# cuMF/cumf_als

Hardware: AMD Instinct MI355X
Metric: ratings/sec per ALS half-iteration (Netflix f=100); RMSE vs reference (higher is better)
Workload: dtype f32 (bf16x3-split products on the bf16 matrix pipe, fp32 accumulate); 1 GPU; netflix-shape synthetic ratings 17770x480189, nnz=99072112, f=100, lambda=0.048, solver=lu, X_BATCH=1 THETA_BATCH=1, fused Gram+solve; step=update-X + update-Theta (two half-iterations)

## Files before the change

cumf_als_amd/csrc/als_internal.h:

```cpp
#ifndef CUMF_ALS_INTERNAL_H_
#define CUMF_ALS_INTERNAL_H_

#include <hip/hip_runtime.h>

#include <algorithm>
#include <cstddef>
#include <type_traits>

#ifndef CUMF_ABLATE
#define CUMF_ABLATE 0
#endif

namespace cumf {

constexpr int kThreads = 256;
constexpr int kStage = 32;
constexpr int kVecLd = 128;
constexpr int kMaxFusedNB = 9;
constexpr int kMaxF = 207;
constexpr int kMaxFAny = 512;
constexpr int kMaxWaveNB = 7;
constexpr int kMaxFusedLuWaveNB = 9;

enum { kModeCG = 0, kModeLU = 1, kModeMaterialize = 2, kModeLUExact = 3, kModeCGHalf = 4 };

__host__ __device__ constexpr int nb_for_f(int f) { return f / 16 + 1; }
constexpr int kMaxNB = nb_for_f(kMaxF);
__host__ __device__ constexpr int solve_ldg(int f, int mode) { return mode == kModeCG ? ((f + 1 + 3) & ~3) : (f + 1); }
__host__ __device__ constexpr size_t solve_g_floats(int f, int mode) {
  return ((size_t)f * solve_ldg(f, mode) + 3) & ~(size_t)3;
}
__host__ __device__ constexpr size_t lu_packed_floats(int nb) { return (size_t)256 * nb * (nb + 1) / 2 + 16 * nb; }
__host__ __device__ constexpr size_t lu_lds_floats(int nb, int f) { return lu_packed_floats(nb) + (size_t)((f + 3) & ~3) + 48; }
constexpr int kCgExtraFloats = 12 * kVecLd;
__host__ __device__ constexpr size_t solve_lds_floats(int f, int mode) {
  return solve_g_floats(f, mode) + (mode == kModeCG ? (size_t)kCgExtraFloats : 0);
}

__host__ __device__ constexpr bool fused_supported(int f, int mode) {
  return mode == kModeLU ? nb_for_f(f) <= nb_for_f(kMaxF) : (f <= kVecLd && nb_for_f(f) <= kMaxFusedNB);
}

struct KernelArgs {
  const int* item_row;
  const long long* item_begin;
  const int* item_len;
  const int* item_slot;
  const int* item_rowlen;
  const int* mrow_row;
  const int* mrow_slot0;
  const int* mrow_nslots;
  const int* mrow_rowlen;
  float* part;
  const int* colidx;
  const float* val;
  const float* gather;
  float* update;
  float* tt;
  float* rhs;
  int tt_half;
  int tt_packed;
  int dense_slots;
  int whole_only;
  long long row_begin;
  int f;
  float lambda;
  int cg_iters;
  int dbg;
  int fast_words;
  int* fast_flag;
  int pre_words;
  unsigned pre_pitch;
  double* sse_bins;
  const float* gather_f32;
  int no_pack;
};
constexpr int kSseBins = 1024;

struct PlanLists {
  long n_items, n_mrows;
  long n_citems, n_witems;
  const int *c_row, *c_len, *c_slot, *c_rowlen;
  const long long* c_begin;
  const int *w_row, *w_len, *w_rowlen;
  const long long* w_begin;
  float* part2;
  long part2_rows;
  double chunk_share;
  long n_short;
};
constexpr int kShortRow = 32;
bool short_cg_available(int f);
hipError_t launch_short_cg(const KernelArgs& a, long n_items, hipStream_t stream);
hipError_t launch_solve_batched(const float* A, const float* b, float* x, long batch, int f, int mode, int cg_iters,
                                hipStream_t stream);
enum { kGramAuto = 0, kGramExact = 1, kGramFast = 2 };
enum { kArithSplit3 = 0, kArithFast = 1, kArithPre = 2, kArithPrePk = 3, kArithSplitPk = 4 };

struct Switches {
  int gram;
  int presplit;
  double presplit_mb;
  bool splitpk;
  bool short_cg;
  bool batched;
  bool wave_solve;
  bool lu_exact;
};
Switches switches();
void set_gram_mode(int mode);
void set_presplit_mode(int mode);

struct PlanFacts {
  int nb;
  long n_mrows, n_citems, n_witems;
  double chunk_share;
  long n_short;
  long gather_rows;
};
enum Path {
  kPathNone,
  kPathGeneric,
  kPathWorkgroup,
  kPathOneWave,
  kPathTwoWave,
};
enum Table { kTableNone, kTablePlanes, kTableF16Words };
enum Solve {
  kSolveInKernel,
  kSolveTileBuffer,
  kSolveReduce,
  kSolveWaveCG,
};
struct Route {
  Path path;
  int arith;
  int fc;
  Table table;
  bool chunk_first;
  long n_short;
  Solve chunked;
  Solve whole;
  bool sse;
};
Route route_for(int f, int mode, const PlanFacts& plan, const Switches& sw);
hipError_t launch_half_iteration(const KernelArgs& a, int mode, const Route& r, const PlanLists& lists, hipStream_t stream);

hipError_t launch_presplit(const float* src, unsigned* dst, size_t n, int* flag, hipStream_t stream);
hipError_t launch_gram_generic(const KernelArgs& a, long n_items, hipStream_t stream);
hipError_t launch_lu_global(float* A, const float* b, float* x, long batch, int f, hipStream_t stream);
__host__ __device__ constexpr bool presplit_supported(int f) {
  return ((nb_for_f(f) == 7 || nb_for_f(f) == 5) && ((f & 15) == 0 || (f & 15) == 4)) ||
         (nb_for_f(f) > kMaxWaveNB && nb_for_f(f) <= nb_for_f(kMaxF) && (f & 3) == 0 && (f & 15) <= 8);
}
__host__ __device__ constexpr bool presplit_pays(int f) { return presplit_supported(f) && nb_for_f(f) >= 7; }
__host__ __device__ constexpr bool presplit_pays_any_size(int f) { return presplit_supported(f) && nb_for_f(f) >= 10; }
__host__ __device__ constexpr unsigned presplit_pitch(int f) {
  return 96u * (f / 16) + ((f & 15) ? (nb_for_f(f) > kMaxWaveNB ? 64u : 32u) : 0u);
}
hipError_t launch_presplit3(const float* src, void* dst, long long rows, int f, hipStream_t stream);
hipError_t launch_pack_upper(const float* full, float* packed, long batch, int f, int unpack, hipStream_t stream);
void set_last_error(int code);
void set_kernel_timing(bool on);
void note_item_kernel(const void* host_function);
const void* last_item_kernel();
hipError_t last_kernel_ms(float* item_ms, float* reduce_ms);
hipError_t kernel_ms_since_reset(float* item_ms, float* reduce_ms, int* launches);
hipError_t launch_quadratic_terms(const float* A, const float* b, const float* x, const float* reg, long batch, int f,
                                  double* out, hipStream_t stream);
hipError_t launch_sse(const float* val, const int* row, const int* col, const float* thetaT, const float* XT,
                      long count, int f, int surpass_nan, double* out, hipStream_t stream);
hipError_t launch_cg_global(const float* A, const float* b, float* x, long batch, int f, int cg_iters, bool a_half,
                            hipStream_t stream);

template <int NB>
hipError_t slice_half_iteration(const KernelArgs& a, int mode, long n_items, long n_mrows, hipStream_t stream);
template <int NB>
hipError_t slice_solve(const float* A, const float* b, float* x, long batch, int f, int mode, int cg_iters,
                       hipStream_t stream);
template <int NB>
hipError_t slice_reduce_only(const KernelArgs& a, int mode, const Route& r, long n_mrows, hipStream_t stream);
template <int NB>
hipError_t slice_batched(const KernelArgs& a, int mode, const Route& r, const PlanLists& L, hipStream_t stream);
template <int NB>
hipError_t wave_item_launch(const KernelArgs& a, int mode, const Route& r, bool whole, long n_items, hipStream_t stream);
template <int NB>
hipError_t wave_solve_launch(const KernelArgs& a, int mode, long n_rows, hipStream_t stream);
template <int NB>
hipError_t wave_lu_launch(const KernelArgs& a, const Route& r, bool whole, long n_items, hipStream_t stream);
template <int NB>
hipError_t wave_cg_hist(unsigned long long* out16);

template <int LO, int HI, class Go>
hipError_t with_nb(int nb, Go&& go) {
  if constexpr (LO > HI)
    return hipErrorInvalidValue;
  else
    return nb == LO ? go(std::integral_constant<int, LO>{}) : with_nb<LO + 1, HI>(nb, go);
}

#define CUMF_LOCAL __attribute__((visibility("hidden")))

enum {
  kScratchTiles = 0,
  kScratchWords = 1,
  kScratchPlanes = 2,
  kScratchImpGram = 3,
  kScratchImpSlots = 4,
  kScratchImpTT = 5,
  kScratchImpRhs = 6,
  kScratchImpX = 7,
  kScratchImpAux = 8,
  kScratchTopkWork = 9,
  kScratchTopkPart = 10,
  kScratchTopkMetrics = 11,
  kScratchNnlsTT = 12,
  kScratchNnlsRhs = 13,
  kScratchRankKeys = 14,
  kScratchRankHist = 15,
  kScratchRankValid = 16,
  kScratchRankMetrics = 17,
};
int scratch_get(hipStream_t stream, int kind, size_t bytes, void** out);
template <typename T>
CUMF_LOCAL inline int scratch(hipStream_t stream, int kind, size_t count, T** out) {
  void* q = nullptr;
  const int rc = scratch_get(stream, kind, (count ? count : 1) * sizeof(T), &q);
  *out = static_cast<T*>(q);
  return rc;
}
CUMF_LOCAL size_t scratch_capacity(hipStream_t stream, int kind);
CUMF_LOCAL int fast_flag_get(int** out);
struct ScratchLease {
  int dev = 0;
  ScratchLease();
  ~ScratchLease();
  ScratchLease(const ScratchLease&) = delete;
  ScratchLease& operator=(const ScratchLease&) = delete;
};
struct ImplicitLists;
void free_implicit_lists(ImplicitLists* lists);

}

struct cumf_plan {
  long rows = 0, row_begin = 0, row_end = 0;
  int f = 0, nb = 0, chunk = 0;
  long long plan_nnz = 0;
  long long chunk_nnz = 0;
  long n_items = 0, n_slots = 0, n_mrows = 0;
  long n_short = 0;
  int* d_item_row = nullptr;
  long long* d_item_begin = nullptr;
  int* d_item_len = nullptr;
  int* d_item_slot = nullptr;
  int* d_item_rowlen = nullptr;
  int* d_mrow_row = nullptr;
  int* d_mrow_slot0 = nullptr;
  int* d_mrow_nslots = nullptr;
  int* d_mrow_rowlen = nullptr;
  float* d_part = nullptr;
  char* d_block = nullptr;
  long n_citems = 0, n_witems = 0;
  int *d_c_row = nullptr, *d_c_len = nullptr, *d_c_slot = nullptr, *d_c_rowlen = nullptr;
  long long* d_c_begin = nullptr;
  int *d_w_row = nullptr, *d_w_len = nullptr, *d_w_rowlen = nullptr;
  long long* d_w_begin = nullptr;
  long gather_rows = 0;
  cumf::ImplicitLists* implicit = nullptr;
};

namespace cumf {

CUMF_LOCAL int plan_lists(const cumf_plan* p, PlanLists* out, hipStream_t stream, bool need_tiles);
CUMF_LOCAL PlanFacts plan_facts(const cumf_plan* p);

template <bool NOTE = false, typename... P, typename... A>
hipError_t launch_kernel(void (*kernel)(P...), dim3 grid, dim3 block, size_t lds, hipStream_t stream, const A&... args) {
  const void* fn = reinterpret_cast<const void*>(kernel);
  if (lds > 64 * 1024) {
    hipError_t e = hipFuncSetAttribute(fn, hipFuncAttributeMaxDynamicSharedMemorySize, (int)lds);
    if (e != hipSuccess) return e;
  }
  if (NOTE) note_item_kernel(fn);
  hipLaunchKernelGGL(kernel, grid, block, lds, stream, args...);
  return hipGetLastError();
}
template <typename... P, typename... A>
hipError_t launch_item_kernel(void (*kernel)(P...), dim3 grid, dim3 block, size_t lds, hipStream_t stream,
                              const A&... args) {
  return launch_kernel<true>(kernel, grid, block, lds, stream, args...);
}

}

#define CUMF_HIP_CHECK(call)                                                                          \
  do {                                                                                                \
    hipError_t err__ = (call);                                                                        \
    if (err__ != hipSuccess) {                                                                        \
      fprintf(stderr, "HIP Error:\nFile = %s\nLine = %d\nReason = %s\n", __FILE__, __LINE__,          \
              hipGetErrorString(err__));                                                              \
      return (int)err__;                                                                              \
    }                                                                                                 \
  } while (0)

#endif
```

cumf_als_amd/csrc/als_launch.cpp:

```cpp
#include <atomic>
#include <mutex>
#include <vector>

#include "als_internal.h"

namespace cumf {

namespace {
struct TimedLaunch {
  hipEvent_t ev[3];
  bool item, reduce;
};
constexpr size_t kTimedPool = 1024;
bool g_timing = false;
std::vector<TimedLaunch> g_timed;
size_t g_timed_used = 0;
TimedLaunch* g_newest = nullptr;
std::mutex g_timed_mutex;

TimedLaunch* timing_begin() {
  if (!g_timing) return nullptr;
  std::lock_guard<std::mutex> lock(g_timed_mutex);
  if (g_timed_used == kTimedPool) g_timed_used = 0;
  g_newest = &g_timed[g_timed_used++];
  return g_newest;
}

std::atomic<const void*> g_last_item_kernel{nullptr};
}

void set_kernel_timing(bool on) {
  std::lock_guard<std::mutex> lock(g_timed_mutex);
  g_timing = on;
  if (on && g_timed.empty()) {
    g_timed.resize(kTimedPool);
    for (auto& t : g_timed) {
      for (auto& e : t.ev) (void)hipEventCreate(&e);
      t.item = t.reduce = false;
    }
  }
}
hipError_t last_kernel_ms(float* item_ms, float* reduce_ms) {
  *item_ms = 0.f;
  *reduce_ms = 0.f;
  const TimedLaunch* t = g_newest;
  if (!t) return hipSuccess;
  hipError_t e = hipEventSynchronize(t->ev[2]);
  if (e != hipSuccess) return e;
  if (t->item) (void)hipEventElapsedTime(item_ms, t->ev[0], t->ev[1]);
  if (t->reduce) (void)hipEventElapsedTime(reduce_ms, t->ev[1], t->ev[2]);
  return hipSuccess;
}
hipError_t kernel_ms_since_reset(float* item_ms, float* reduce_ms, int* launches) {
  std::lock_guard<std::mutex> lock(g_timed_mutex);
  *item_ms = 0.f;
  *reduce_ms = 0.f;
  *launches = (int)g_timed_used;
  for (size_t i = 0; i < g_timed_used; ++i) {
    TimedLaunch& t = g_timed[i];
    hipError_t e = hipEventSynchronize(t.ev[2]);
    if (e != hipSuccess) return e;
    float ms = 0.f;
    if (t.item && hipEventElapsedTime(&ms, t.ev[0], t.ev[1]) == hipSuccess) *item_ms += ms;
    if (t.reduce && hipEventElapsedTime(&ms, t.ev[1], t.ev[2]) == hipSuccess) *reduce_ms += ms;
  }
  g_timed_used = 0;
  return hipSuccess;
}

void note_item_kernel(const void* host_function) { g_last_item_kernel.store(host_function, std::memory_order_relaxed); }
const void* last_item_kernel() { return g_last_item_kernel.load(std::memory_order_relaxed); }

static hipError_t wave_items(const KernelArgs& a, int mode, const Route& r, bool whole, long n_items, hipStream_t stream) {
  return with_nb<2, kMaxWaveNB>(nb_for_f(a.f), [&](auto nb) { return wave_item_launch<nb>(a, mode, r, whole, n_items, stream); });
}

static hipError_t one_wave_items(const KernelArgs& a, int mode, const Route& r, const PlanLists& L, hipStream_t stream) {
  KernelArgs aw = a;
  long n_items = L.n_items;
  if (r.chunk_first) {
    aw.item_row = L.w_row, aw.item_begin = L.w_begin, aw.item_len = L.w_len;
    aw.item_slot = nullptr, aw.item_rowlen = L.w_rowlen;
    n_items = L.n_witems;
  }
  if (r.n_short > 0) {
    n_items -= r.n_short;
    KernelArgs as = aw;
    as.item_row += n_items, as.item_begin += n_items, as.item_len += n_items, as.item_rowlen += n_items;
    hipError_t e = launch_short_cg(as, r.n_short, stream);
    if (e != hipSuccess) return e;
  }
  if (r.chunk_first) {
    KernelArgs ac = a;
    ac.item_row = L.c_row, ac.item_begin = L.c_begin, ac.item_len = L.c_len;
    ac.item_slot = L.c_slot, ac.item_rowlen = L.c_rowlen;
    hipError_t e = wave_items(ac, mode, r, false, L.n_citems, stream);
    if (e != hipSuccess) return e;
  }
  return wave_items(aw, mode, r, r.chunk_first || L.n_mrows == 0, n_items, stream);
}

hipError_t launch_half_iteration(const KernelArgs& a, int mode, const Route& r, const PlanLists& L, hipStream_t stream) {
  const int nb = nb_for_f(a.f);
  TimedLaunch* t = timing_begin();
  if (t) {
    t->item = r.path == kPathTwoWave || L.n_items > 0;
    t->reduce = r.path != kPathTwoWave && L.n_mrows > 0;
    (void)hipEventRecord(t->ev[0], stream);
  }
  hipError_t e = hipErrorInvalidValue;
  switch (r.path) {
    case kPathTwoWave:
      e = with_nb<kMaxWaveNB + 1, kMaxNB>(nb, [&](auto n) { return slice_batched<n>(a, mode, r, L, stream); });
      break;
    case kPathOneWave: e = one_wave_items(a, mode, r, L, stream); break;
    case kPathWorkgroup:
      e = with_nb<1, kMaxNB>(nb, [&](auto n) { return slice_half_iteration<n>(a, mode, L.n_items, 0, stream); });
      break;
    default: break;
  }
  if (t) (void)hipEventRecord(t->ev[1], stream);
  if (e == hipSuccess && r.path != kPathTwoWave && L.n_mrows > 0) {
    e = with_nb<1, kMaxNB>(nb, [&](auto n) {
      return r.path == kPathOneWave ? slice_reduce_only<n>(a, mode, r, L.n_mrows, stream)
                                    : slice_half_iteration<n>(a, mode, 0, L.n_mrows, stream);
    });
  }
  if (t) (void)hipEventRecord(t->ev[2], stream);
  return e;
}

hipError_t launch_solve_batched(const float* A, const float* b, float* x, long batch, int f, int mode, int cg_iters,
                                hipStream_t stream) {
  if (batch <= 0) return hipSuccess;
  if (mode == kModeLUExact) return slice_solve<0>(A, b, x, batch, f, mode, 0, stream);
  if (f > 128 && (mode == kModeCG || mode == kModeCGHalf))
    return launch_cg_global(A, b, x, batch, f, cg_iters, mode == kModeCGHalf, stream);
  return with_nb<1, kMaxNB>(nb_for_f(f), [&](auto n) { return slice_solve<n>(A, b, x, batch, f, mode, cg_iters, stream); });
}

}
```

cumf_als_amd/csrc/als_plan.cpp:

```cpp
#include <hip/hip_runtime.h>

#include <algorithm>
#include <cstdint>
#include <cstdio>
#include <cstdlib>
#include <numeric>
#include <vector>

#include "als_internal.h"
#include "cumf_als_capi.h"

using namespace cumf;

namespace {

int default_chunk(int f, long long nnz) {
  (void)f;
  const char* e = getenv("CUMF_ALS_CHUNK");
  int c;
  if (e) {
    c = atoi(e);
  } else {
    int cus = 256;
    int dev = 0;
    if (hipGetDevice(&dev) == hipSuccess) (void)hipDeviceGetAttribute(&cus, hipDeviceAttributeMultiprocessorCount, dev);
    const long long slots = (long long)(cus > 0 ? cus : 256) * 4;
    const long long want = nnz / (slots * 12);
    c = (int)std::min<long long>(8192, std::max<long long>(2048, want));
  }
  if (c < kStage) c = kStage;
  return (c / kStage) * kStage;
}

}

extern "C" int cumf_plan_create(cumf_plan_t** out, const void* rowptr_host, int rowptr_is_64, long rows,
                                long row_begin, long row_end, int f, int chunk) {
  if (!out || !rowptr_host || rows < 0 || row_begin < 0 || row_end > rows || row_begin > row_end) {
    fprintf(stderr, "cumf_plan_create: invalid arguments\n");
    return (int)hipErrorInvalidValue;
  }
  if (f <= 0 || f > kMaxFAny || (f % 2) != 0) {
    fprintf(stderr, "cumf_plan_create: f = %d unsupported (need even f <= %d)\n", f, kMaxFAny);
    return (int)hipErrorInvalidValue;
  }
  auto rp = [&](long i) -> long long {
    return rowptr_is_64 ? static_cast<const long long*>(rowptr_host)[i]
                        : static_cast<long long>(static_cast<const int*>(rowptr_host)[i]);
  };
  if (chunk <= 0) chunk = default_chunk(f, rp(rows) - rp(0));
  if (f > kMaxF) {
    long long longest = 0;
    for (long u = row_begin; u < row_end; ++u) longest = std::max(longest, rp(u + 1) - rp(u));
    chunk = (int)std::min<long long>(0x7fffffe0LL, std::max<long long>(longest, kStage));
    chunk = ((chunk + kStage - 1) / kStage) * kStage;
  }
  chunk = std::max(kStage, (chunk / kStage) * kStage);

  std::vector<int> item_row, item_len, item_slot, item_rowlen;
  std::vector<long long> item_begin;
  std::vector<int> mrow_row, mrow_slot0, mrow_nslots, mrow_rowlen;
  {
    const size_t guess = (size_t)(row_end - row_begin) + (size_t)((rp(row_end) - rp(row_begin)) / chunk) + 16;
    item_row.reserve(guess), item_len.reserve(guess), item_slot.reserve(guess), item_rowlen.reserve(guess);
    item_begin.reserve(guess);
  }
  long n_slots = 0;
  for (long u = row_begin; u < row_end; ++u) {
    const long long s = rp(u), e = rp(u + 1);
    const long long len = e - s;
    if (len < 0 || len > 0x7fffffffLL) {
      fprintf(stderr, "cumf_plan_create: row %ld has invalid length %lld\n", u, len);
      return (int)hipErrorInvalidValue;
    }
    if (len <= chunk) {
      item_row.push_back((int)u);
      item_begin.push_back(s);
      item_len.push_back((int)len);
      item_slot.push_back(-1);
      item_rowlen.push_back((int)len);
    } else {
      const int nchunks = len == 0 ? 1 : (int)((len + chunk - 1) / chunk);
      mrow_row.push_back((int)u);
      mrow_slot0.push_back((int)n_slots);
      mrow_nslots.push_back(nchunks);
      mrow_rowlen.push_back((int)len);
      for (int c = 0; c < nchunks; ++c) {
        const long long b = s + (long long)c * chunk;
        item_row.push_back((int)u);
        item_begin.push_back(b);
        item_len.push_back((int)std::max<long long>(0, std::min<long long>(chunk, e - b)));
        item_slot.push_back((int)(n_slots + c));
        item_rowlen.push_back((int)len);
      }
      n_slots += nchunks;
    }
  }
  const size_t n_it = item_row.size();
  std::vector<long> order(n_it);
  static const int order_mode = getenv("CUMF_ALS_ORDER") ? atoi(getenv("CUMF_ALS_ORDER")) : 0;
  long n_short = 0;
  if (order_mode == 0) {
    auto bucket = [&](size_t i) -> size_t {
      const bool is_short = item_slot[i] < 0 && item_len[i] <= kShortRow;
      return is_short ? (size_t)chunk + 1 + (size_t)(kShortRow - item_len[i]) : (size_t)(chunk - item_len[i]);
    };
    std::vector<long> start((size_t)chunk + kShortRow + 3, 0);
    for (size_t i = 0; i < n_it; ++i) {
      ++start[bucket(i) + 1];
      n_short += item_slot[i] < 0 && item_len[i] <= kShortRow;
    }
    for (size_t k = 1; k < start.size(); ++k) start[k] += start[k - 1];
    for (size_t i = 0; i < n_it; ++i) order[(size_t)start[bucket(i)]++] = (long)i;
  } else {
    std::iota(order.begin(), order.end(), 0L);
  }

  cumf_plan* p = new cumf_plan();
  p->rows = rows;
  p->row_begin = row_begin;
  p->row_end = row_end;
  p->f = f;
  p->nb = nb_for_f(f);
  p->chunk = chunk;
  p->plan_nnz = rp(row_end) - rp(row_begin);
  p->n_items = (long)n_it;
  p->n_short = n_short;
  p->n_slots = n_slots;
  p->n_mrows = (long)mrow_row.size();
  for (size_t i = 0; i < n_it; ++i) {
    if (item_slot[i] >= 0) {
      ++p->n_citems;
      p->chunk_nnz += item_len[i];
    }
  }
  p->n_witems = p->n_items - p->n_citems;
  *out = nullptr;

  const size_t ni = n_it, nm = mrow_row.size(), nc = (size_t)p->n_citems, nw = (size_t)p->n_witems;
  size_t off = 0;
  auto piece = [&](size_t count, size_t elem) {
    const size_t at = off;
    off += (count * elem + 255) & ~(size_t)255;
    return at;
  };
  const size_t o_item_row = piece(ni, 4), o_item_begin = piece(ni, 8), o_item_len = piece(ni, 4), o_item_slot = piece(ni, 4),
               o_item_rowlen = piece(ni, 4), o_mrow_row = piece(nm, 4), o_mrow_slot0 = piece(nm, 4),
               o_mrow_nslots = piece(nm, 4), o_mrow_rowlen = piece(nm, 4), o_c_row = piece(nc, 4), o_c_begin = piece(nc, 8),
               o_c_len = piece(nc, 4), o_c_slot = piece(nc, 4), o_c_rowlen = piece(nc, 4), o_w_row = piece(nw, 4),
               o_w_begin = piece(nw, 8), o_w_len = piece(nw, 4), o_w_rowlen = piece(nw, 4);
  std::vector<char> host(off ? off : 256);
  auto ints = [&](size_t o) { return reinterpret_cast<int*>(host.data() + o); };
  auto longs = [&](size_t o) { return reinterpret_cast<long long*>(host.data() + o); };
  {
    size_t ic = 0, iw = 0;
    for (size_t k = 0; k < ni; ++k) {
      const size_t i = (size_t)order[k];
      ints(o_item_row)[k] = item_row[i];
      longs(o_item_begin)[k] = item_begin[i];
      ints(o_item_len)[k] = item_len[i];
      ints(o_item_slot)[k] = item_slot[i];
      ints(o_item_rowlen)[k] = item_rowlen[i];
      if (item_slot[i] >= 0) {
        ints(o_c_row)[ic] = item_row[i];
        longs(o_c_begin)[ic] = item_begin[i];
        ints(o_c_len)[ic] = item_len[i];
        ints(o_c_slot)[ic] = item_slot[i];
        ints(o_c_rowlen)[ic] = item_rowlen[i];
        ++ic;
      } else {
        ints(o_w_row)[iw] = item_row[i];
        longs(o_w_begin)[iw] = item_begin[i];
        ints(o_w_len)[iw] = item_len[i];
        ints(o_w_rowlen)[iw] = item_rowlen[i];
        ++iw;
      }
    }
    for (size_t k = 0; k < nm; ++k) {
      ints(o_mrow_row)[k] = mrow_row[k];
      ints(o_mrow_slot0)[k] = mrow_slot0[k];
      ints(o_mrow_nslots)[k] = mrow_nslots[k];
      ints(o_mrow_rowlen)[k] = mrow_rowlen[k];
    }
  }
#define PLAN_CHECK(call)                                                                                    \
  do {                                                                                                      \
    hipError_t err__ = (call);                                                                              \
    if (err__ != hipSuccess) {                                                                              \
      fprintf(stderr, "HIP Error:\nFile = %s\nLine = %d\nReason = %s\n", __FILE__, __LINE__,              \
              hipGetErrorString(err__));                                                                    \
      cumf_plan_destroy(p);                              \
      return (int)err__;                                                                                    \
    }                                                                                                       \
  } while (0)
  PLAN_CHECK(hipMalloc(reinterpret_cast<void**>(&p->d_block), host.size()));
  PLAN_CHECK(hipMemcpy(p->d_block, host.data(), host.size(), hipMemcpyHostToDevice));
  auto dints = [&](size_t o, size_t count) { return count ? reinterpret_cast<int*>(p->d_block + o) : nullptr; };
  auto dlongs = [&](size_t o, size_t count) { return count ? reinterpret_cast<long long*>(p->d_block + o) : nullptr; };
  p->d_item_row = dints(o_item_row, ni), p->d_item_begin = dlongs(o_item_begin, ni), p->d_item_len = dints(o_item_len, ni);
  p->d_item_slot = dints(o_item_slot, ni), p->d_item_rowlen = dints(o_item_rowlen, ni);
  p->d_mrow_row = dints(o_mrow_row, nm), p->d_mrow_slot0 = dints(o_mrow_slot0, nm);
  p->d_mrow_nslots = dints(o_mrow_nslots, nm), p->d_mrow_rowlen = dints(o_mrow_rowlen, nm);
  p->d_c_row = dints(o_c_row, nc), p->d_c_begin = dlongs(o_c_begin, nc), p->d_c_len = dints(o_c_len, nc);
  p->d_c_slot = dints(o_c_slot, nc), p->d_c_rowlen = dints(o_c_rowlen, nc);
  p->d_w_row = dints(o_w_row, nw), p->d_w_begin = dlongs(o_w_begin, nw), p->d_w_len = dints(o_w_len, nw);
  p->d_w_rowlen = dints(o_w_rowlen, nw);
  if (n_slots > 0) {
    const size_t tiles = (size_t)p->nb * (p->nb + 1) / 2;
    PLAN_CHECK(hipMalloc(reinterpret_cast<void**>(&p->d_part), (size_t)n_slots * tiles * 256 * sizeof(float)));
  }
#undef PLAN_CHECK
  *out = p;
  return 0;
}

extern "C" int cumf_plan_destroy(cumf_plan_t* p) {
  if (!p) return 0;
  if (p->d_block) (void)hipFree(p->d_block);
  if (p->d_part) (void)hipFree(p->d_part);
  free_implicit_lists(p->implicit);
  delete p;
  return 0;
}

extern "C" int cumf_plan_set_gather_rows(cumf_plan_t* p, long gather_rows) {
  if (!p || gather_rows < 0) return (int)hipErrorInvalidValue;
  p->gather_rows = gather_rows;
  return 0;
}

extern "C" int cumf_plan_info(const cumf_plan_t* p, long info[4]) {
  if (!p || !info) return (int)hipErrorInvalidValue;
  info[0] = p->n_items;
  info[1] = p->n_slots;
  info[2] = p->n_mrows;
  info[3] = p->chunk;
  return 0;
}

int cumf::plan_lists(const cumf_plan_t* p, PlanLists* out, hipStream_t stream, bool need_tiles) {
  const size_t tile_bytes = (size_t)p->nb * (p->nb + 1) / 2 * 256 * sizeof(float);
  float* part2 = nullptr;
  long rows = 0;
  if (need_tiles && p->n_witems > 0) {
    static const double cap_gb = getenv("CUMF_ALS_TILE_BUFFER_GB") ? atof(getenv("CUMF_ALS_TILE_BUFFER_GB")) : 48.0;
    size_t cap = (size_t)(cap_gb * (double)(1ull << 30));
    size_t free_b = 0, total_b = 0;
    if (hipMemGetInfo(&free_b, &total_b) == hipSuccess) {
      const size_t mine = scratch_capacity(stream, kScratchTiles);
      cap = std::min(cap, (free_b + mine) / 2);
    }
    if (cap < ((size_t)2 << 30)) cap = (size_t)2 << 30;
    rows = (long)std::min<size_t>((size_t)p->n_witems, cap / tile_bytes);
    if (rows < 1) rows = 1;
    void* q = nullptr;
    const int rc = scratch_get(stream, kScratchTiles, (size_t)rows * tile_bytes, &q);
    if (rc) return rc;
    part2 = static_cast<float*>(q);
  }
  *out = PlanLists{p->n_items,  p->n_mrows, p->n_citems, p->n_witems, p->d_c_row,    p->d_c_len,  p->d_c_slot,
                   p->d_c_rowlen, p->d_c_begin, p->d_w_row,  p->d_w_len,  p->d_w_rowlen, p->d_w_begin, part2,
                   rows,          p->plan_nnz > 0 ? (double)p->chunk_nnz / (double)p->plan_nnz : 0.0, p->n_short};
  return 0;
}

PlanFacts cumf::plan_facts(const cumf_plan_t* p) {
  return PlanFacts{p->nb, p->n_mrows, p->n_citems, p->n_witems,
                   p->plan_nnz > 0 ? (double)p->chunk_nnz / (double)p->plan_nnz : 0.0, p->n_short, p->gather_rows};
}
```

cumf_als_amd/csrc/als_route.cpp:

```cpp
#include <cstdlib>

#include "als_internal.h"
#include "cumf_als_capi.h"

namespace cumf {

namespace {
int g_gram_mode = -1;
int g_presplit_mode = -2;
}

void set_gram_mode(int mode) { g_gram_mode = (mode == kGramExact || mode == kGramFast) ? mode : kGramAuto; }
void set_presplit_mode(int mode) { g_presplit_mode = mode; }

Switches switches() {
  if (g_gram_mode < 0) {
    const char* e = getenv("CUMF_ALS_GRAM");
    g_gram_mode = (e && (e[0] == 'e' || e[0] == 'E')) ? kGramExact : (e && (e[0] == 'f' || e[0] == 'F')) ? kGramFast : kGramAuto;
  }
  if (g_presplit_mode == -2) {
    const char* e = getenv("CUMF_ALS_PRESPLIT");
    g_presplit_mode = (e && e[0] == '0') ? CUMF_PRESPLIT_OFF : (e && e[0] == '1') ? CUMF_PRESPLIT_ON
                      : (e && e[0] == '2') ? CUMF_PRESPLIT_VERIFY : CUMF_PRESPLIT_AUTO;
  }
  static const double presplit_mb = getenv("CUMF_ALS_PRESPLIT_MB") ? atof(getenv("CUMF_ALS_PRESPLIT_MB")) : 64.0;
  static const bool splitpk = !(getenv("CUMF_ALS_SPLITPK") && *getenv("CUMF_ALS_SPLITPK") == '0');
  static const bool short_cg = !getenv("CUMF_ALS_SHORT_CG") || atoi(getenv("CUMF_ALS_SHORT_CG")) != 0;
  const char* lu_exact = getenv("CUMF_ALS_LU_EXACT");
  return Switches{g_gram_mode,
                  g_presplit_mode,
                  presplit_mb,
                  splitpk,
                  short_cg,
                  !getenv("CUMF_ALS_NO_BATCHED"),
                  !getenv("CUMF_ALS_NO_WAVE_SOLVE"),
                  lu_exact && atoi(lu_exact) != 0};
}

static bool presplit_wanted(int f, long gather_rows, const Switches& sw) {
  if (sw.presplit == CUMF_PRESPLIT_OFF || sw.gram != kGramAuto || !presplit_supported(f) || gather_rows <= 0) return false;
  if (sw.presplit == CUMF_PRESPLIT_ON || sw.presplit == CUMF_PRESPLIT_VERIFY) return true;
  return presplit_pays_any_size(f) || (presplit_pays(f) && (double)gather_rows * presplit_pitch(f) <= sw.presplit_mb * 1048576.0);
}

Route route_for(int f, int mode, const PlanFacts& p, const Switches& sw) {
  Route r{};
  const int nb = nb_for_f(f);
  const bool wave_gram = sw.gram != kGramExact;
  if (f > kMaxF)
    r.path = mode == kModeMaterialize ? kPathGeneric : kPathNone;
  else if (wave_gram && nb >= 2 && nb <= kMaxWaveNB)
    r.path = kPathOneWave;
  else if (wave_gram && sw.batched && nb > kMaxWaveNB)
    r.path = kPathTwoWave;
  else
    r.path = (mode == kModeMaterialize || fused_supported(f, mode)) ? kPathWorkgroup : kPathNone;
  const bool one = r.path == kPathOneWave, wave = one || r.path == kPathTwoWave;

  r.arith = kArithSplit3;
  if (wave && mode != kModeMaterialize) {
    if (sw.gram == kGramFast) {
      r.table = kTableF16Words;
      r.arith = kArithFast;
    } else if (presplit_wanted(f, p.gather_rows, sw)) {
      r.table = kTablePlanes;
      r.arith = (one && sw.presplit != CUMF_PRESPLIT_VERIFY) ? kArithPrePk : kArithPre;
    } else if (one && sw.splitpk && (f & 15) == 0 && sw.presplit != CUMF_PRESPLIT_OFF &&
               sw.presplit != CUMF_PRESPLIT_VERIFY) {
      r.arith = kArithSplitPk;
    }
  }
  r.fc = (one && f == 100) ? 100 : 0;

  r.chunked = (wave && mode == kModeCG && sw.wave_solve && (one || f > kVecLd)) ? kSolveWaveCG : kSolveReduce;
  r.whole = (r.path == kPathTwoWave && mode != kModeCG && !(mode == kModeLU && nb <= kMaxFusedLuWaveNB)) ? kSolveTileBuffer
                                                                                                          : kSolveInKernel;
  r.chunk_first = one && mode == kModeLU && p.n_mrows > 0 && p.n_citems > 0 && p.n_witems > 0 && p.chunk_share < 0.25;
  r.n_short = (one && mode == kModeCG && sw.short_cg && short_cg_available(f)) ? p.n_short : 0;
  r.sse = wave && mode != kModeMaterialize &&
          (p.n_mrows == 0 || r.chunked == kSolveWaveCG || (mode == kModeLU && nb >= 7));
  return r;
}

}
```

Before: 12.26 billion ratings/s.

## Solve short rows via dual n×n system instead of f×f normal equations

```diff
diff --git a/cumf_als_amd/csrc/als_dual.hip b/cumf_als_amd/csrc/als_dual.hip
--- /dev/null
+++ b/cumf_als_amd/csrc/als_dual.hip
@@ -0,0 +1,159 @@
+#include <hip/hip_runtime.h>
+
+#define CUMF_WAVE_NB 8
+#define CUMF_WAVE_PART 2
+#include "als_wave.hip"
+
+namespace cumf {
+
+namespace {
+
+constexpr int kDualVec = 128;
+template <int NBD>
+__host__ __device__ constexpr int dual_lds_floats() { return wave_lu_lds_floats<NBD>(16 * NBD - 1) + kDualVec; }
+
+typedef __attribute__((address_space(1))) const u32x4 g_u32x4;
+typedef __attribute__((address_space(1))) const u32x2 g_u32x2;
+typedef __attribute__((address_space(1))) const f32x2 g_f32x2;
+typedef __attribute__((address_space(1))) const float g_float;
+template <class T>
+__device__ __forceinline__ T* as_global(const void* p) { return reinterpret_cast<T*>(reinterpret_cast<unsigned long long>(p)); }
+
+template <int NBD, bool PRE>
+__global__ __launch_bounds__(64, 3) void als_dual_kernel(const KernelArgs a) {
+  extern __shared__ __attribute__((aligned(16))) float smem[];
+  constexpr int NT = NBD * (NBD + 1) / 2;
+  const int lane = threadIdx.x, c = lane & 15, g = lane >> 4;
+  const int item = blockIdx.x;
+  const int row = a.item_row[item];
+  const long long begin = a.item_begin[item];
+  const int n = a.item_len[item];
+  const int f = a.f;
+  float* xg = a.update + (size_t)row * f;
+  if (n <= 0) {
+    const float nan = __builtin_nanf("");
+    if (lane < f) xg[lane] = nan;
+    if (lane + 64 < f) xg[lane + 64] = nan;
+    return;
+  }
+  const int fsys = n < 16 * (NBD - 1) ? 16 * (NBD - 1) : n;
+  float* vec = smem + wave_lu_lds_floats<NBD>(16 * NBD - 1);
+  vec[lane] = lane < n ? a.val[begin + lane] : 0.f;
+  vec[lane + 64] = lane + 64 < n ? a.val[begin + lane + 64] : 0.f;
+
+  const char* trow[NBD];
+#pragma unroll
+  for (int I = 0; I < NBD; ++I) {
+    const int i = 16 * I + c;
+    const int j = i < n ? a.colidx[begin + i] : -1;
+    const char* base = PRE ? reinterpret_cast<const char*>(a.gather) + (size_t)j * a.pre_pitch
+                           : reinterpret_cast<const char*>(a.gather_f32 + (size_t)j * f);
+    trow[I] = j >= 0 ? base : nullptr;
+  }
+
+  f32x4 acc[NT];
+#pragma unroll
+  for (int t = 0; t < NT; ++t) acc[t] = f32x4{0.f, 0.f, 0.f, 0.f};
+
+  const int fb16 = 16 * (f >> 4);
+  const int nslab = (f + 31) >> 5;
+  for (int s = 0; s < nslab; ++s) {
+    const int k0 = 32 * s + 8 * g;
+    u32x4 H[NBD], M[NBD], L[NBD];
+#pragma unroll
+    for (int I = 0; I < NBD; ++I) {
+      H[I] = M[I] = L[I] = u32x4{0u, 0u, 0u, 0u};
+      if (trow[I] == nullptr) continue;
+      if constexpr (PRE) {
+        if (k0 + 8 <= fb16) {
+          const char* p = trow[I] + 2 * k0;
+          H[I] = *as_global<g_u32x4>(p);
+          M[I] = *as_global<g_u32x4>(p + 2 * fb16);
+          L[I] = *as_global<g_u32x4>(p + 4 * fb16);
+        } else if (k0 == fb16 && fb16 < f) {
+          const char* p = trow[I] + 6 * fb16;
+          const u32x2 h = *as_global<g_u32x2>(p), m = *as_global<g_u32x2>(p + 8),
+                      l = *as_global<g_u32x2>(p + 16);
+          H[I] = u32x4{h[0], h[1], 0u, 0u};
+          M[I] = u32x4{m[0], m[1], 0u, 0u};
+          L[I] = u32x4{l[0], l[1], 0u, 0u};
+        }
+      } else {
+#pragma unroll
+        for (int e = 0; e < 4; ++e) {
+          f32x2 v = {0.f, 0.f};
+          if (k0 + 2 * e < f) v = *as_global<g_f32x2>(trow[I] + 4 * (k0 + 2 * e));
+          unsigned h, m, l;
+          split3_pair(v[0], v[1], h, m, l);
+          H[I][e] = h, M[I][e] = m, L[I][e] = l;
+        }
+      }
+    }
+    static_for<NT>([&](auto tc) {
+      constexpr int t = decltype(tc)::value, I = tile_I<NBD>(t), J = tile_J<NBD>(t);
+      acc[t] = mfma_bf16(L[I], H[J], acc[t]);
+      acc[t] = mfma_bf16(H[I], L[J], acc[t]);
+      acc[t] = mfma_bf16(M[I], M[J], acc[t]);
+      acc[t] = mfma_bf16(M[I], H[J], acc[t]);
+      acc[t] = mfma_bf16(H[I], M[J], acc[t]);
+      acc[t] = mfma_bf16(H[I], H[J], acc[t]);
+    });
+  }
+
+  __syncthreads();
+  const int cn = fsys - 16 * (NBD - 1);
+  static_for<NBD>([&](auto ic) {
+    constexpr int I = decltype(ic)::value, t = tile_of<NBD>(I, NBD - 1);
+    const f32x4 rv = *reinterpret_cast<const f32x4*>(vec + 16 * I + 4 * g);
+    if (c == cn) acc[t] = rv;
+  });
+  const float reg = (float)n * a.lambda;
+  __syncthreads();
+  const float ssq = lu_wave_blocked<NBD, 0>(acc, smem, fsys, reg, vec, lane);
+  __syncthreads();
+
+  const bool f0 = lane < f, f1 = lane + 64 < f;
+  float x0 = 0.f, x1 = 0.f;
+#pragma unroll 16
+  for (int i = 0; i < n; ++i) {
+    g_float* t = as_global<g_float>(a.gather_f32 + (size_t)a.colidx[begin + i] * f);
+    const float y = vec[i];
+    const float t0 = f0 ? t[lane] : 0.f, t1 = f1 ? t[lane + 64] : 0.f;
+    x0 = fmaf(t0, y, x0);
+    x1 = fmaf(t1, y, x1);
+  }
+  if (f0) xg[lane] = x0;
+  if (f1) xg[lane + 64] = x1;
+  if (a.sse_bins != nullptr) {
+    const float yy = wave_sum_uniform(ssq);
+    wave_sse_add(a.sse_bins, (double)reg * (double)reg * (double)yy, n, lane);
+  }
+}
+
+template <int NBD>
+hipError_t launch_dual_nbd(const KernelArgs& a, long n_items, bool note, hipStream_t stream) {
+  const size_t lds = dual_lds_floats<NBD>() * sizeof(float);
+  const auto kernel = a.pre_pitch != 0 ? als_dual_kernel<NBD, true> : als_dual_kernel<NBD, false>;
+  return note ? launch_item_kernel(kernel, dim3((unsigned)n_items), dim3(64), lds, stream, a)
+              : launch_kernel(kernel, dim3((unsigned)n_items), dim3(64), lds, stream, a);
+}
+
+}
+
+hipError_t launch_dual(const KernelArgs& a, const long (&count)[kDualClasses], bool note, hipStream_t stream) {
+  if (a.f < kDualMinF || nb_for_f(a.f) > kMaxWaveNB) return hipErrorInvalidValue;
+  KernelArgs d = a;
+  for (int k = 0; k < kDualClasses; ++k) {
+    const long cnt = count[k];
+    if (cnt <= 0) continue;
+    hipError_t e = k == 0   ? launch_dual_nbd<5>(d, cnt, note, stream)
+                   : k == 1 ? launch_dual_nbd<4>(d, cnt, note, stream)
+                   : k == 2 ? launch_dual_nbd<3>(d, cnt, note, stream)
+                            : launch_dual_nbd<2>(d, cnt, note, stream);
+    if (e != hipSuccess) return e;
+    d.item_row += cnt, d.item_begin += cnt, d.item_len += cnt, d.item_rowlen += cnt;
+  }
+  return hipSuccess;
+}
+
+}
diff --git a/cumf_als_amd/csrc/als_internal.h b/cumf_als_amd/csrc/als_internal.h
--- a/cumf_als_amd/csrc/als_internal.h
+++ b/cumf_als_amd/csrc/als_internal.h
@@ -88,10 +88,15 @@
   long part2_rows;
   double chunk_share;
   long n_short;
+  long n_dual[4];
 };
 constexpr int kShortRow = 32;
 bool short_cg_available(int f);
 hipError_t launch_short_cg(const KernelArgs& a, long n_items, hipStream_t stream);
+constexpr int kDualMaxRow = 79;
+constexpr int kDualClasses = 4;
+constexpr int kDualMinF = 32;
+hipError_t launch_dual(const KernelArgs& a, const long (&count)[kDualClasses], bool note, hipStream_t stream);
 hipError_t launch_solve_batched(const float* A, const float* b, float* x, long batch, int f, int mode, int cg_iters,
                                 hipStream_t stream);
 enum { kGramAuto = 0, kGramExact = 1, kGramFast = 2 };
@@ -106,6 +111,7 @@
   bool batched;
   bool wave_solve;
   bool lu_exact;
+  bool dual;
 };
 Switches switches();
 void set_gram_mode(int mode);
@@ -117,6 +123,7 @@
   double chunk_share;
   long n_short;
   long gather_rows;
+  long n_dual;
 };
 enum Path {
   kPathNone,
@@ -139,6 +146,7 @@
   Table table;
   bool chunk_first;
   long n_short;
+  bool dual;
   Solve chunked;
   Solve whole;
   bool sse;
@@ -250,6 +258,7 @@
   long long chunk_nnz = 0;
   long n_items = 0, n_slots = 0, n_mrows = 0;
   long n_short = 0;
+  long n_dual[cumf::kDualClasses] = {0, 0, 0, 0};
   int* d_item_row = nullptr;
   long long* d_item_begin = nullptr;
   int* d_item_len = nullptr;
diff --git a/cumf_als_amd/csrc/als_launch.cpp b/cumf_als_amd/csrc/als_launch.cpp
--- a/cumf_als_amd/csrc/als_launch.cpp
+++ b/cumf_als_amd/csrc/als_launch.cpp
@@ -90,6 +90,15 @@
     hipError_t e = launch_short_cg(as, r.n_short, stream);
     if (e != hipSuccess) return e;
   }
+  if (r.dual && a.lambda > 0.f) {
+    const long n_dual = L.n_dual[0] + L.n_dual[1] + L.n_dual[2] + L.n_dual[3];
+    n_items -= n_dual;
+    KernelArgs ad = aw;
+    ad.item_row += n_items, ad.item_begin += n_items, ad.item_len += n_items, ad.item_rowlen += n_items;
+    if (r.table != kTablePlanes) ad.pre_pitch = 0;
+    hipError_t e = launch_dual(ad, L.n_dual, n_items == 0 && !r.chunk_first, stream);
+    if (e != hipSuccess) return e;
+  }
   if (r.chunk_first) {
     KernelArgs ac = a;
     ac.item_row = L.c_row, ac.item_begin = L.c_begin, ac.item_len = L.c_len;
diff --git a/cumf_als_amd/csrc/als_plan.cpp b/cumf_als_amd/csrc/als_plan.cpp
--- a/cumf_als_amd/csrc/als_plan.cpp
+++ b/cumf_als_amd/csrc/als_plan.cpp
@@ -126,6 +126,15 @@
   p->plan_nnz = rp(row_end) - rp(row_begin);
   p->n_items = (long)n_it;
   p->n_short = n_short;
+  if (order_mode == 0 && f >= kDualMinF) {
+    static const int env_max = getenv("CUMF_ALS_DUAL_MAX") ? atoi(getenv("CUMF_ALS_DUAL_MAX")) : kDualMaxRow;
+    const int dual_max = std::min(std::min(f - 1, kDualMaxRow), env_max);
+    for (size_t i = 0; i < n_it; ++i) {
+      if (item_slot[i] >= 0 || item_len[i] > dual_max) continue;
+      const int cls = item_len[i] >= 64 ? 0 : item_len[i] >= 48 ? 1 : item_len[i] >= 32 ? 2 : 3;
+      ++p->n_dual[cls];
+    }
+  }
   p->n_slots = n_slots;
   p->n_mrows = (long)mrow_row.size();
   for (size_t i = 0; i < n_it; ++i) {
@@ -260,11 +269,13 @@
   }
   *out = PlanLists{p->n_items,  p->n_mrows, p->n_citems, p->n_witems, p->d_c_row,    p->d_c_len,  p->d_c_slot,
                    p->d_c_rowlen, p->d_c_begin, p->d_w_row,  p->d_w_len,  p->d_w_rowlen, p->d_w_begin, part2,
-                   rows,          p->plan_nnz > 0 ? (double)p->chunk_nnz / (double)p->plan_nnz : 0.0, p->n_short};
+                   rows,          p->plan_nnz > 0 ? (double)p->chunk_nnz / (double)p->plan_nnz : 0.0, p->n_short,
+                   {p->n_dual[0], p->n_dual[1], p->n_dual[2], p->n_dual[3]}};
   return 0;
 }
 
 PlanFacts cumf::plan_facts(const cumf_plan_t* p) {
   return PlanFacts{p->nb, p->n_mrows, p->n_citems, p->n_witems,
-                   p->plan_nnz > 0 ? (double)p->chunk_nnz / (double)p->plan_nnz : 0.0, p->n_short, p->gather_rows};
-}
+                   p->plan_nnz > 0 ? (double)p->chunk_nnz / (double)p->plan_nnz : 0.0, p->n_short, p->gather_rows,
+                   p->n_dual[0] + p->n_dual[1] + p->n_dual[2] + p->n_dual[3]};
+}
diff --git a/cumf_als_amd/csrc/als_route.cpp b/cumf_als_amd/csrc/als_route.cpp
--- a/cumf_als_amd/csrc/als_route.cpp
+++ b/cumf_als_amd/csrc/als_route.cpp
@@ -27,6 +27,7 @@
   static const bool splitpk = !(getenv("CUMF_ALS_SPLITPK") && *getenv("CUMF_ALS_SPLITPK") == '0');
   static const bool short_cg = !getenv("CUMF_ALS_SHORT_CG") || atoi(getenv("CUMF_ALS_SHORT_CG")) != 0;
   const char* lu_exact = getenv("CUMF_ALS_LU_EXACT");
+  const char* dual = getenv("CUMF_ALS_DUAL");
   return Switches{g_gram_mode,
                   g_presplit_mode,
                   presplit_mb,
@@ -34,7 +35,8 @@
                   short_cg,
                   !getenv("CUMF_ALS_NO_BATCHED"),
                   !getenv("CUMF_ALS_NO_WAVE_SOLVE"),
-                  lu_exact && atoi(lu_exact) != 0};
+                  lu_exact && atoi(lu_exact) != 0,
+                  !(dual && (dual[0] == 'o' || dual[0] == 'O' || dual[0] == '0'))};
 }
 
 static bool presplit_wanted(int f, long gather_rows, const Switches& sw) {
@@ -77,6 +79,8 @@
                                                                                                           : kSolveInKernel;
   r.chunk_first = one && mode == kModeLU && p.n_mrows > 0 && p.n_citems > 0 && p.n_witems > 0 && p.chunk_share < 0.25;
   r.n_short = (one && mode == kModeCG && sw.short_cg && short_cg_available(f)) ? p.n_short : 0;
+  r.dual = one && mode == kModeLU && sw.dual && sw.gram == kGramAuto && sw.presplit != CUMF_PRESPLIT_VERIFY &&
+           f >= kDualMinF && p.n_dual > 0;
   r.sse = wave && mode != kModeMaterialize &&
           (p.n_mrows == 0 || r.chunked == kSolveWaveCG || (mode == kModeLU && nb >= 7));
   return r;
```

Result: slower. 12.12 billion ratings/s (-1.2%).
